# medical-genomics-group/rs-bann

Hardware: AMD Instinct MI355X
Metric: HMC leapfrog steps/sec (whole node), 50k indiv × 500k SNP × 1k branches (higher is better)
Workload: dtype 2-bit genotype codes x f32 params (i8 MFMA digits, exact int32 accumulate, f32 head); 1 GPU; c3: 1000 branches x 500 SNPs, n=50000, D=1 W=4 S=4, RidgeARD, tanh, Izmailov step sizes; n=50000, snps=500000, branches=1000, branches_per_gpu=1000, parallelism=branch-shard x1

## Files before the change

include/bann.h:

```cpp
#ifndef BANN_H
#define BANN_H

#include <stdint.h>

#ifdef __cplusplus
extern "C" {
#endif

typedef struct bann_ctx bann_ctx;

typedef enum {
  BANN_OK = 0,
  BANN_E_HIP = -1,
  BANN_E_SHAPE = -2,
  BANN_E_OOM = -3,
  BANN_E_STATE = -4,
  BANN_E_ARG = -5
} bann_status;

typedef enum { BANN_TANH = 0, BANN_RELU = 1, BANN_LEAKY_RELU = 2, BANN_SILU = 3, BANN_IDENTITY = 4 } bann_activation;

typedef enum {
  BANN_RIDGE_ARD = 0,
  BANN_RIDGE_BASE = 1,
// ... 136 lines not shown
int bann_residual_to_target(bann_ctx* ctx, int32_t b);
int bann_residual_from_target(bann_ctx* ctx, int32_t b, double* sum, double* sumsq);
int bann_rebuild_targets(bann_ctx* ctx, const int32_t* branches, int32_t nb, const float* residual_device);


int bann_gibbs_posterior(bann_ctx* ctx, const int32_t* branches, int32_t nb, const float* hyper, double* shape_out,
                         double* scale_out, double* out_stat_out);
int bann_gibbs_sample_precisions(bann_ctx* ctx, const int32_t* branches, int32_t nb, const float* hyper,
                                 float output_precision, float error_precision, uint64_t seed);
int bann_get_params_all(bann_ctx* ctx, float* out);


int bann_arch_layer_widths(int32_t m, int32_t depth, int32_t hidden_rule, int32_t hidden_fixed, float hidden_fraction,
                           int32_t summary_rule, int32_t summary_fixed, float summary_fraction,
                           int32_t* layer_widths_out);

typedef struct {
  int32_t mode;
  float variance, gamma_shape, gamma_scale;
  int32_t num_effective;
  float proportion_effective;
  int32_t has_fixed_precision;  float fixed_precision;
} bann_init_cfg;
int bann_init_branches(bann_ctx* ctx, const int32_t* branches, int32_t nb, const bann_init_cfg* cfg, uint64_t seed);


typedef int (*bann_allreduce_fn)(void* user, void* host_buf, int64_t count, int32_t dtype);

int bann_shard_branches(const int32_t* marker_counts, int32_t nbranches, int32_t world, int32_t* starts_out);
int bann_comm_unique_id(uint8_t* id_out);
int bann_ctx_comm_init(bann_ctx* ctx, const uint8_t* id, int32_t nranks, int32_t rank);
int bann_ctx_comm_callback(bann_ctx* ctx, bann_allreduce_fn fn, void* user, int32_t nranks, int32_t rank);
int bann_comm_info(const bann_ctx* ctx, int32_t* kind, int32_t* nranks, int32_t* rank, int32_t* backend_ranks);
int bann_residual_update_host(bann_allreduce_fn fn, void* user, float* local_delta, float* residual, int64_t n);
int bann_exchange_residual(bann_ctx* ctx, float* residual_host);
int bann_exchange_residual_device(bann_ctx* ctx);
int bann_network_hmc_step(bann_ctx* ctx, const float* y, float bias, float lambda_e, int32_t L,
                          float max_hamiltonian_error, int32_t step_mode, float step_factor, const float* eps,
                          const float* momentum, uint64_t seed, const float* u, int32_t* status_out,
                          double* h_trace_out, double* rss_out);
int bann_set_network_step_rule(bann_ctx* ctx, int32_t common_mode, float tau);
int bann_set_network_adapt_trajectories(bann_ctx* ctx, int32_t k);
int bann_network_step_rule_state(const bann_ctx* ctx, int32_t* mode, int32_t* adapted, int32_t* frozen);
int bann_network_info(const bann_ctx* ctx, int32_t* group_rows);
int bann_network_step_rule_info(const bann_ctx* ctx, double* out4);

int bann_branch_kernel_path(const bann_ctx* ctx, int32_t b);
const char* bann_fused_kernel_name(void);
int bann_set_hidden_gemm_bf16(bann_ctx* ctx, int32_t enabled);
int bann_set_graph_replay(bann_ctx* ctx, int32_t enabled);
int bann_get_graph_replay(const bann_ctx* ctx);
int bann_set_fused_enabled(bann_ctx* ctx, int32_t enabled);
int64_t bann_packed_genotype_bytes(const bann_ctx* ctx);

#ifdef __cplusplus
}
#endif
#endif
```

rs-bann_amd/bann/_lib.py:

```python
from __future__ import annotations

import ctypes as C
import os

HERE = os.path.dirname(os.path.abspath(__file__))
PKG_ROOT = os.path.dirname(HERE)
REPO_ROOT = os.path.dirname(PKG_ROOT)
LIB_PATH = os.environ.get("BANN_LIB") or os.path.join(PKG_ROOT, "librsbann_amd.so")
HEADER_PATH = os.path.join(REPO_ROOT, "include", "bann.h")
HEADER_PATHS = [HEADER_PATH, os.path.join(REPO_ROOT, "include", "bann_net.h")]

BANN_OK = 0
STATUS = {0: "BANN_OK", -1: "BANN_E_HIP", -2: "BANN_E_SHAPE", -3: "BANN_E_OOM", -4: "BANN_E_STATE",
          -5: "BANN_E_ARG"}
ACTIVATIONS = {"tanh": 0, "relu": 1, "leaky_relu": 2, "silu": 3, "identity": 4}
PRIORS = {"ridge_ard": 0, "ridge_base": 1, "lasso_ard": 2, "lasso_base": 3, "std_normal": 4}
STEP_MODES = {"uniform": 0, "random": 1, "std_scaled": 2, "izmailov": 3, "injected": 100}
HMC_STATUS = {0: "accepted", 1: "rejected", 2: "rejected_early"}


class BannLibraryError(RuntimeError):
    pass


# ... 115 lines not shown
    "bann_exchange_residual_device": (C.c_int, [_P]),
    "bann_set_network_step_rule": (C.c_int, [_P, _i32, _f32]),
    "bann_network_step_rule_info": (C.c_int, [_P, _pf64]),
    "bann_set_network_adapt_trajectories": (C.c_int, [_P, _i32]),
    "bann_network_info": (C.c_int, [_P, C.POINTER(C.c_int32)]),
    "bann_network_step_rule_state": (C.c_int, [_P, C.POINTER(C.c_int32), C.POINTER(C.c_int32), C.POINTER(C.c_int32)]),
    "bann_residual_set": (C.c_int, [_P, _pf32]),
    "bann_residual_get": (C.c_int, [_P, _pf32]),
    "bann_residual_device": (C.c_int, [_P, C.POINTER(_pf32)]),
    "bann_residual_init": (C.c_int, [_P, _pf32, _f32, _pf64, _pf64]),
    "bann_residual_stats": (C.c_int, [_P, _pf64, _pf64]),
    "bann_residual_shift": (C.c_int, [_P, _f32, _pf64, _pf64]),
    "bann_residual_to_target": (C.c_int, [_P, _i32]),
    "bann_residual_from_target": (C.c_int, [_P, _i32, _pf64, _pf64]),
    "bann_rebuild_targets": (C.c_int, [_P, _pi32, _i32, _P]),
    "bann_set_launch_timing": (C.c_int, [_P, _i32]),
    "bann_launch_timing": (C.c_int, [_P, _pf32, _pf32, _pi32, _i32]),
    "bann_network_timing": (C.c_int, [_P, _pf32, _pf32, _pi32, _i32]),
    "bann_ctx_num_individuals": (_i64, [_P]),
    "bann_leapfrog_begin": (C.c_int, [_P, _pi32, _i32, _i32, _f32, _i32, _f32, _u64]),
    "bann_leapfrog_steps": (C.c_int, [_P, _i32]),
    "bann_leapfrog_end": (C.c_int, [_P, _pi32, _pi32]),
    "bann_leapfrog_predictions_device": (C.c_int, [_P, C.POINTER(_pf32)]),
    "bann_leapfrog_residual_delta_device": (C.c_int, [_P, _P]),
    "bann_leapfrog_residual_delta": (C.c_int, [_P, _P]),
    "bann_fused_kernel_name": (C.c_char_p, []),
    "bann_branch_get_step_sizes": (C.c_int, [_P, C.c_int32, _P]),
    "bann_predict_many": (C.c_int, [_P, _P, C.c_int32, _P]),
    "bann_synchronize": (C.c_int, [_P]),
    "bann_gibbs_posterior": (C.c_int, [_P, _pi32, _i32, _pf32, _pf64, _pf64, _pf64]),
    "bann_gibbs_sample_precisions": (C.c_int, [_P, _pi32, _i32, _pf32, _f32, _f32, _u64]),
    "bann_get_params_all": (C.c_int, [_P, _pf32]),
    "bann_arch_layer_widths": (C.c_int, [_i32, _i32, _i32, _i32, _f32, _i32, _i32, _f32, _pi32]),
    "bann_init_branches": (C.c_int, [_P, _pi32, _i32, C.POINTER(InitCfg), _u64]),
    "bann_phen_stats_write": (C.c_int, [C.c_char_p, _f32, _f32, _f32]),
    "bann_net_init": (C.c_int, [_P, C.POINTER(InitCfg), _u64]),
    "bann_net_simulate_y": (C.c_int, [_P, _P, _f32, _u64, _pf32, _pf32]),
    "bann_net_write_params": (C.c_int, [_P, C.c_char_p]),
    "bann_models_reserve": (C.c_int, [_P, _i32]),
    "bann_models_capacity": (C.c_int, [_P]),
    "bann_models_pass_width": (C.c_int, []),
    "bann_models_set_params": (C.c_int, [_P, _i32, _i32, _pf32]),
    "bann_models_set_bias": (C.c_int, [_P, _i32, _f32]),
    "bann_models_predict": (C.c_int, [_P, _i32, _i32, _pf32, _pf32, _pf32]),
    "bann_models_branch_predictions": (C.c_int, [_P, _i32, _pi32, _i32, _pf32]),
    "bann_models_stats_pass_width": (C.c_int, []),
    "bann_models_branch_stats": (C.c_int, [_P, _i32, _i32, _pi32, _i32, _pf32, _pf64, _pf32, _pf32, _pf32]),
    "bann_models_branch_stats_timed": (C.c_int, [_P, _i32, _i32, _pi32, _i32, _pf32, _pf64, _pf32, _pf32]),
    "bann_profile_session": (C.c_int, [_P, _i32, _pf32, _pf32]),
    "bann_branch_kernel_path": (C.c_int, [_P, _i32]),
    "bann_set_fused_enabled": (C.c_int, [_P, _i32]),
    "bann_set_hidden_gemm_bf16": (C.c_int, [_P, _i32]),
    "bann_packed_genotype_bytes": (_i64, [_P]),
    "bann_net_create": (C.c_int, [_P, C.POINTER(PrecisionHyperparams), _u64, C.POINTER(_P)]),
    "bann_net_destroy": (C.c_int, [_P]),
    "bann_net_set_rng_hooks": (C.c_int, [_P, C.POINTER(RngHooks)]),
    "bann_net_set_global": (C.c_int, [_P, _f32, _f32, _f32, _f32]),
    "bann_net_train": (C.c_int, [_P, _pf32, _i64, C.POINTER(McmcCfg), C.c_char_p]),
    "bann_net_train_single_branch": (C.c_int, [_P, _pf32, _i64, C.POINTER(McmcCfg), C.c_char_p]),
    "bann_net_train_network": (C.c_int, [_P, _pf32, _i64, C.POINTER(McmcCfg), _i32, C.c_char_p]),
    "bann_net_network_timing": (C.c_int, [_P, _pf64]),
    "bann_net_perturb": (C.c_int, [_P, _i32, _f32, _i32, _f32]),
    "bann_net_predict": (C.c_int, [_P, _P, _pf32]),
    "bann_net_predict_models": (C.c_int, [_P, _P, C.POINTER(C.c_char_p), _i32, _pf32, _pf32, _pf32]),
    "bann_net_rss": (C.c_int, [_P, _P, _pf32, _i64, _pf64]),
    "bann_net_gradient": (C.c_int, [_P, _P, _pf32, _i64, _pf32]),
    "bann_net_branch_r2s": (C.c_int, [_P, _P, _pf32, _i64, _pf32]),
    "bann_net_activations": (C.c_int, [_P, _P, _i32, _pf32]),
    "bann_net_population_effect_sizes": (C.c_int, [_P, _P, _pf32]),
    "bann_net_branch_r2s_models": (C.c_int, [_P, _P, C.POINTER(C.c_char_p), _i32, _pf32, _i64, _pf32]),
    "bann_net_population_effect_sizes_models": (C.c_int, [_P, _P, C.POINTER(C.c_char_p), _i32, _pf32, _pf32, _pf32]),
    "bann_net_summary": (C.c_int, [_P, C.POINTER(TrainSummary)]),
    "bann_net_records": (C.c_int, [_P, _pf32, _pf32, _i32]),
    "bann_net_residual": (C.c_int, [_P, _pf32]),
    "bann_net_set_test_data": (C.c_int, [_P, _P, _pf32, _i64]),
    "bann_net_records_test": (C.c_int, [_P, _pf32, _i32]),
    "bann_set_trajectory_recording": (C.c_int, [_P, _i32]),
    "bann_branch_get_trajectory": (C.c_int, [_P, _i32, _i32, _pi32, _pf32, _pf32, _pf64]),
    "bann_branch_get_trajectory_joint": (C.c_int, [_P, _i32, _i32, _pi32, _pf32, _pf32, _pf32, _pf64]),
    "bann_set_graph_replay": (C.c_int, [_P, _i32]),
    "bann_get_graph_replay": (C.c_int, [_P]),
    "bann_net_save": (C.c_int, [_P, C.c_char_p]),
    "bann_net_load": (C.c_int, [_P, C.c_char_p]),
    "bann_net_last_error": (C.c_char_p, [_P]),
}

_lib = None


def load_library(path: str = LIB_PATH):
    global _lib
    if _lib is not None:
        return _lib
    if not os.path.exists(path):
        raise BannLibraryError(
            f"{path} not found: build the HIP library first (python -c 'import __graft_entry__ as g; g.build()' "
            "or make -C rs-bann_amd/csrc).  There is no CPU fallback.")
    lib = C.CDLL(path)
    for name, (res, args) in SIGNATURES.items():
        fn = getattr(lib, name)
        fn.restype = res
        fn.argtypes = args
    _lib = lib
    return lib
```

rs-bann_amd/csrc/kernel_util.h:

```cpp
#pragma once
#include <hip/hip_runtime.h>
#include <stdint.h>

#include "bann_internal.h"

typedef int v4i __attribute__((ext_vector_type(4)));
typedef float v4f __attribute__((ext_vector_type(4)));

struct HeadLds {
  float W[BANN_MAXL][4][4];
  float bias[BANN_MAXL][4];
};

__device__ __forceinline__ float wave_sum(float v) {
#pragma unroll
  for (int o = 32; o > 0; o >>= 1) v += __shfl_xor(v, o);
  return v;
}
__device__ __forceinline__ double wave_sum_d(double v) {
#pragma unroll
  for (int o = 32; o > 0; o >>= 1) v += __shfl_xor(v, o);
  return v;
}

#define LDS_BARRIER()                                      \
  do {                                                     \
    asm volatile("s_waitcnt lgkmcnt(0)" ::: "memory");     \
    __builtin_amdgcn_s_barrier();                          \
    asm volatile("" ::: "memory");                         \
  } while (0)

typedef __attribute__((address_space(3))) void* lds_ptr_t;

__device__ __forceinline__ uint32_t lds_off(const void* p) { return (uint32_t)(uintptr_t)p; }
__device__ __forceinline__ void glds16(const void* gsrc, const void* lds_dst) {
  const uint32_t m0 = __builtin_amdgcn_readfirstlane(lds_off(lds_dst));
#ifndef BANN_GLDS_NT
#define BANN_GLDS_NT 1
#endif
#if BANN_GLDS_NT
  asm volatile("s_mov_b32 m0, %0\n\ts_nop 0\n\tglobal_load_lds_dwordx4 %1, off nt" ::"s"(m0), "v"(gsrc) : "memory", "m0");
#else
  asm volatile("s_mov_b32 m0, %0\n\ts_nop 0\n\tglobal_load_lds_dwordx4 %1, off" ::"s"(m0), "v"(gsrc) : "memory", "m0");
#endif
}
__device__ __forceinline__ void glds16_s(const void* sbase, uint32_t voff, const void* lds_dst) {
  const uint32_t m0 = __builtin_amdgcn_readfirstlane(lds_off(lds_dst));
#if BANN_GLDS_NT
  asm volatile("s_mov_b32 m0, %0\n\ts_nop 0\n\tglobal_load_lds_dwordx4 %1, %2 nt" ::"s"(m0), "v"(voff), "s"(sbase)
               : "memory", "m0");
#else
  asm volatile("s_mov_b32 m0, %0\n\ts_nop 0\n\tglobal_load_lds_dwordx4 %1, %2" ::"s"(m0), "v"(voff), "s"(sbase)
               : "memory", "m0");
#endif
}
__device__ __forceinline__ void glds4(const void* gsrc, const void* lds_dst) {
  const uint32_t m0 = __builtin_amdgcn_readfirstlane(lds_off(lds_dst));
  asm volatile("s_mov_b32 m0, %0\n\ts_nop 0\n\tglobal_load_lds_dword %1, off" ::"s"(m0), "v"(gsrc) : "memory", "m0");
}
__device__ __forceinline__ void lds_st_f32(float* p, float v) {
  asm volatile("ds_write_b32 %0, %1" ::"v"(lds_off(p)), "v"(v) : "memory");
}
__device__ __forceinline__ void lds_st_v4f(v4f* p, v4f v) {
  asm volatile("ds_write_b128 %0, %1" ::"v"(lds_off(p)), "v"(v) : "memory");
}

__device__ __forceinline__ uint32_t fbits(float x) { return __builtin_bit_cast(uint32_t, x); }
__device__ __forceinline__ float fpow2(uint32_t biased_exp) { return __builtin_bit_cast(float, biased_exp << 23); }

typedef unsigned short v2u16 __attribute__((ext_vector_type(2)));
__device__ __forceinline__ uint32_t max_u16x2(uint32_t a, uint32_t b) {
  return __builtin_bit_cast(uint32_t, __builtin_elementwise_max(__builtin_bit_cast(v2u16, a), __builtin_bit_cast(v2u16, b)));
}
__device__ __forceinline__ uint32_t wave_max_u16x2(uint32_t v) {
  v = max_u16x2(v, (uint32_t)__builtin_amdgcn_update_dpp((int)v, (int)v, 0xB1, 0xF, 0xF, false));
  v = max_u16x2(v, (uint32_t)__builtin_amdgcn_update_dpp((int)v, (int)v, 0x4E, 0xF, 0xF, false));
  v = max_u16x2(v, (uint32_t)__builtin_amdgcn_update_dpp((int)v, (int)v, 0x141, 0xF, 0xF, false));
  v = max_u16x2(v, (uint32_t)__builtin_amdgcn_update_dpp((int)v, (int)v, 0x140, 0xF, 0xF, false));
  v = max_u16x2(v, (uint32_t)__builtin_amdgcn_update_dpp((int)v, (int)v, 0x142, 0xA, 0xF, false));
  v = max_u16x2(v, (uint32_t)__builtin_amdgcn_update_dpp((int)v, (int)v, 0x143, 0xC, 0xF, false));
  return (uint32_t)__builtin_amdgcn_readlane((int)v, 63);
}

typedef int v2i __attribute__((ext_vector_type(2)));
typedef __attribute__((address_space(3))) v2i lds_v2i;
__device__ __forceinline__ v4i lds_tr8_pair(const char* p0, const char* p1) {
  const v2i a = __builtin_amdgcn_ds_read_tr8_b64_v2i32((lds_v2i*)(p0));
  const v2i b = __builtin_amdgcn_ds_read_tr8_b64_v2i32((lds_v2i*)(p1));
  return v4i{a.x, a.y, b.x, b.y};
}

__device__ __forceinline__ uint32_t digits4(float v) {
  uint32_t w = 0;
#pragma unroll
  for (int d = 0; d < 4; ++d) {
    const float r = __builtin_rintf(v);
    w |= ((uint32_t)(int)r & 0xFFu) << (8 * d);
    v = (v - r) * 128.f;
  }
  return w;
}
```

rs-bann_amd/csrc/kernels_fx.hip:

```cpp
#include <stdlib.h>
#include <type_traits>

#include "activations.h"
#include "bann_internal.h"
#include "fx_shapes.h"
#include "kernel_util.h"
#include "update_core.h"

#define FX_WAVES 4
#define FX_SLOT 8192

#ifndef FX_STAMPS
#define FX_STAMPS 0
#endif
#ifndef FXT_PD
#define FXT_PD 12
#endif
#ifndef FX_ABL
#define FX_ABL 0
#endif
#if FX_STAMPS
#define FX_STAMP(i)                                            \
  do {                                                         \
    const unsigned long long t_ = __builtin_amdgcn_s_memtime(); \
    ph[i] += t_ - t_last;                                      \
    t_last = t_;                                               \
  } while (0)
#else
#define FX_STAMP(i) \
  do {              \
  } while (0)
#endif
#if FX_ABL & 8
#define FX_MFMA(a, b, c) ((c) + ((a) ^ (b)))
#else
#define FX_MFMA(a, b, c) __builtin_amdgcn_mfma_i32_16x16x64_i8((a), (b), (c), 0, 0, 0)
#endif

typedef unsigned int v4u __attribute__((ext_vector_type(4)));

#define FX_ONES3 (v4i{0, 0, 0, 0x40404040})

__device__ __forceinline__ void fx_fwd_chunk(v4i A, v4u X, v4i (&facc)[4]) {
  facc[0] = __builtin_amdgcn_mfma_i32_16x16x64_i8(A, (v4i)(X & 0x03030303u), facc[0], 0, 0, 0);
  facc[1] = __builtin_amdgcn_mfma_i32_16x16x64_i8(A, (v4i)(X & 0x0F0F0F0Fu), facc[1], 0, 0, 0);
  facc[2] = __builtin_amdgcn_mfma_i32_16x16x64_i8(A, (v4i)(X & 0x3F3F3F3Fu), facc[2], 0, 0, 0);
  facc[3] = __builtin_amdgcn_mfma_i32_16x16x64_i8(A, (v4i)X, facc[3], 0, 0, 0);
}
__device__ __forceinline__ void fx_fwd_fields(v4i (&facc)[4]) {
  facc[3] -= facc[2];
  facc[2] -= facc[1];
  facc[1] -= facc[0];
}
__device__ __forceinline__ v4i fx_rowsum64_acc(v4i A, v4i acc) {
  return __builtin_amdgcn_mfma_i32_16x16x64_i8(A, v4i{0x40404040, 0x40404040, 0x40404040, 0x40404040}, acc, 0, 0, 0);
}
__device__ __forceinline__ v4i fx_bwd_unpack(uint32_t wv) {
  return v4i{(int)(wv & 0x03030303u), (int)(wv & 0x0C0C0C0Cu), (int)(wv & 0x30303030u), (int)(wv & 0xC0C0C0C0u)};
}

__device__ __forceinline__ float ufl(float v) {
  return __builtin_bit_cast(float, __builtin_amdgcn_readfirstlane(__builtin_bit_cast(int, v)));
}

__device__ __forceinline__ void vm_wait(int k) {
  switch (k) {
    case 2: asm volatile("s_waitcnt vmcnt(2)" ::: "memory"); break;
    case 3: asm volatile("s_waitcnt vmcnt(3)" ::: "memory"); break;
    case 4: asm volatile("s_waitcnt vmcnt(4)" ::: "memory"); break;
    case 5: asm volatile("s_waitcnt vmcnt(5)" ::: "memory"); break;
    case 6: asm volatile("s_waitcnt vmcnt(6)" ::: "memory"); break;
    case 7: asm volatile("s_waitcnt vmcnt(7)" ::: "memory"); break;
// ... 52 lines not shown
                    int32_t* __restrict__ upd_cnt, const FoldJob* __restrict__ folds) {
  constexpr int NH = NL - 1;
  constexpr int NW = FX_WAVES;
  constexpr int NS = 8 + (NH - 1) * 20;
  __shared__ __attribute__((aligned(16))) char s_x[NW][2][FX_SLOT];
  __shared__ __attribute__((aligned(16))) char s_dig[NW][4 * FX_DROW];
  __shared__ __attribute__((aligned(16))) float s_y[NW][2][64];
  __shared__ __attribute__((aligned(16))) char s_w0[8 * 1024];
  __shared__ __attribute__((aligned(16))) float s_hw[NL][20];
  __shared__ float s_hs[NW][NS];
  __shared__ double s_rss[NW];

  const GradItem it = items[blockIdx.x];
  const int b = it.branch;
  const BranchDev& bd = st.br[b];
  const int wave = __builtin_amdgcn_readfirstlane(threadIdx.x >> 6);
  const int lane = threadIdx.x & 63;
  const int nch = NCH ? NCH : bd.nchunks;
  const int64_t n = st.n;
  const int tb = it.frag_begin >> 2, te = (it.frag_end + 3) >> 2;

  const int g = lane >> 4, i16 = lane & 15, tq = i16 >> 1, tp = lane & 1;
  const int gsw = g & 1;
  const uint32_t fo0 = (uint32_t)((16 * g + tq + 8 * gsw) * 16 + 8 * (tp ^ gsw));
  const uint32_t fo1 = (uint32_t)((16 * g + tq + 8 * (1 ^ gsw)) * 16 + 8 * (tp ^ 1 ^ gsw));
  const int pe = i16, po = (i16 + 8) & 15;
  const uint32_t boe = (uint32_t)(pe * 16 + 4 * (2 * ((g >> 1) ^ (pe >> 3)) + (g & 1)));
  const uint32_t boo = (uint32_t)(po * 16 + 4 * (2 * ((g >> 1) ^ (po >> 3)) + (g & 1)));
  const int iota = 4 * i16 + g;
  char* const sd = &s_dig[wave][0];
  char* const sd_w = sd + (i16 >> 2) * FX_DROW + (4 * g + (i16 & 3)) * 16;
  const char* const sd_r = sd + g * FX_DROW + tq * 16 + 8 * tp;
  const bool net_err = st.nete != nullptr;
  const float* ybr = net_err ? st.nete : st.y + bd.y_off;
  float* predb = st.pred + bd.y_off;
  const int64_t tile_bytes = (int64_t)nch * 1024;
  const uint64_t xb = (uint64_t)(uintptr_t)(reinterpret_cast<const char*>(st.xu2) + bd.x_off);
  const char* xbase_s = reinterpret_cast<const char*>(
      ((uint64_t)(uint32_t)__builtin_amdgcn_readfirstlane((int)(uint32_t)(xb >> 32)) << 32) |
      (uint32_t)__builtin_amdgcn_readfirstlane((int)(uint32_t)xb));

  const bool pad_row = 64 * (nch - 1) + 16 * (lane >> 4) + (((lane & 15) - 8 * ((lane >> 4) & 1)) & 15) >= bd.m;
  auto issue_chunk = [&](int tt, int sl, int c) {
    if (FX_ABL & 16) return;
    if (c == nch - 1 && pad_row) return;
    glds16_s(xbase_s + (uint64_t)tt * (uint64_t)tile_bytes + (uint64_t)(c * 1024), (uint32_t)lane * 16u,
             &s_x[wave][sl][c * 1024]);
  };
  auto issue_y = [&](int tt, int sl) {
    if (FX_ABL & 16) return;
    const int64_t row = 64 * (int64_t)tt + iota;
    glds4(ybr + (row < n ? row : n - 1), &s_y[wave][sl][0]);
  };
  int tt = tb + wave, sl = 0;
  if (tt < te) {
    for (int c = 0; c < nch; ++c) issue_chunk(tt, 0, c);
    issue_y(tt, 0);
    if (tt + NW < te) {
      for (int c = 0; c < nch; ++c) issue_chunk(tt + NW, 1, c);
      issue_y(tt + NW, 1);
    }
  }
  const float* th = st.theta + bd.p_off;
  for (int t = threadIdx.x; t < NL * 20; t += 64 * NW) {
    const int l = t / 20, r = t - l * 20;
    float v = 0.f;
    if (r < 16) {
      const int j = r >> 2, k = r & 3;
      if (l >= 1 && j < bd.win[l] && k < bd.widths[l]) v = th[bd.woff[l] + k * bd.win[l] + j];
    } else {
      const int k = r - 16;
      if (l == 0 && k < bd.widths[0]) v = st.fc[b].c0[k];
      if (l >= 1 && l < NH && k < bd.widths[l]) v = th[bd.boff[l] + k];
    }
    s_hw[l][r] = v;
  }
  float zscale = st.fc[b].scale[g];
  for (int c = wave; c < nch; c += NW)
    *reinterpret_cast<v4i*>(&s_w0[c * 1024 + lane * 16]) =
        *reinterpret_cast<const v4i*>(st.dig + bd.dig_off + ((int64_t)c * 64 + lane) * 16);
  asm volatile("s_waitcnt vmcnt(0)" ::: "memory");
  asm volatile("" : "+v"(zscale));
  __syncthreads();
  v4i rowsum64 = v4i{0, 0, 0, 0};
  for (int c = 0; c < nch; ++c) rowsum64 = fx_rowsum64_acc(*reinterpret_cast<const v4i*>(&s_w0[c * 1024 + lane * 16]), rowsum64);
  float uW[NL][4][4], uB[NH][4];
#pragma unroll
  for (int l = 0; l < NL; ++l) {
#pragma unroll
    for (int j = 0; j < 4; ++j)
#pragma unroll
      for (int k = 0; k < 4; ++k)
        uW[l][j][k] = (l >= 1 && (l < NL - 1 || k == 0)) ? sgpr_f(s_hw[l][4 * j + k]) : 0.f;
    if (l < NH)
#pragma unroll
      for (int k = 0; k < 4; ++k) uB[l][k] = sgpr_f(s_hw[l][16 + k]);
  }


  v4i acc[32];
#pragma unroll
  for (int u = 0; u < 32; ++u) acc[u] = v4i{0, 0, 0, 0};
  v4i acc3 = v4i{0, 0, 0, 0};
  int R[4] = {0, 0, 0, 0};
  double rss = 0.0;
  float db[NH][4], dWo[4];
  float dW[NL > 2 ? NL - 2 : 1][4][4];
#pragma unroll
  for (int k = 0; k < 4; ++k) {
    dWo[k] = 0.f;
#pragma unroll
    for (int l = 0; l < NH; ++l) db[l][k] = 0.f;
#pragma unroll
    for (int l = 0; l < (NL > 2 ? NL - 2 : 1); ++l)
#pragma unroll
      for (int j = 0; j < 4; ++j) dW[l][j][k] = 0.f;
  }

#if FX_STAMPS
  unsigned long long ph[8] = {0, 0, 0, 0, 0, 0, 0, 0}, ntl = 0;
  const unsigned long long rt0 = __builtin_amdgcn_s_memrealtime(), mt0 = __builtin_amdgcn_s_memtime();
  unsigned long long t_last = mt0;
#endif
  for (; tt < te; tt += NW, sl ^= 1) {
    const bool more = tt + NW < te;
    const bool more2 = tt + 2 * NW < te;
    FX_STAMP(5);
    vm_wait(more ? nch + 1 : 0);
    FX_STAMP(0);
    const char* xs = &s_x[wave][sl][0];

    v4i facc[4] = {v4i{0, 0, 0, 0}, v4i{0, 0, 0, 0}, v4i{0, 0, 0, 0}, rowsum64};
    __builtin_amdgcn_s_setprio(1);
    {
      constexpr int FD = 2;
      v4u Xq[FD];
      v4i Aq[FD];
#pragma unroll
      for (int c = 0; c < FD; ++c) {
        Xq[c] = v4u{0u, 0u, 0u, 0u};
        Aq[c] = v4i{0, 0, 0, 0};
        if (NCH != 0 || c < nch) {
          Xq[c] = (v4u)lds_tr8_pair(xs + c * 1024 + fo0, xs + c * 1024 + fo1);
          Aq[c] = *reinterpret_cast<const v4i*>(&s_w0[c * 1024 + lane * 16]);
        }
      }
#pragma unroll
      for (int c = 0; c < 8; ++c) {
        if (NCH == 0 && c >= nch) continue;
        const v4u Xc = Xq[c % FD];
        const v4i Ac = Aq[c % FD];
        if (c + FD < 8 && (NCH != 0 || c + FD < nch)) {
          Xq[c % FD] = (v4u)lds_tr8_pair(xs + (c + FD) * 1024 + fo0, xs + (c + FD) * 1024 + fo1);
          Aq[c % FD] = *reinterpret_cast<const v4i*>(&s_w0[(c + FD) * 1024 + lane * 16]);
        }
#if FX_ABL & 1
        const v4i B0 = (v4i)Xc, B1 = (v4i)Xc, B2 = (v4i)Xc, B3 = (v4i)Xc;
#else
        const v4i B0 = (v4i)(Xc & 0x03030303u);
        const v4i B1 = (v4i)(Xc & 0x0F0F0F0Fu);
        const v4i B2 = (v4i)(Xc & 0x3F3F3F3Fu);
        const v4i B3 = (v4i)Xc;
#endif
        facc[0] = FX_MFMA(Ac, B0, facc[0]);
        facc[1] = FX_MFMA(Ac, B1, facc[1]);
        facc[2] = FX_MFMA(Ac, B2, facc[2]);
        facc[3] = FX_MFMA(Ac, B3, facc[3]);
        __builtin_amdgcn_sched_barrier(0);
      }
    }
    __builtin_amdgcn_sched_barrier(0);
    FX_STAMP(1);
    __builtin_amdgcn_s_setprio(1);
    fx_fwd_fields(facc);
    float z0 = zscale * comb4(facc[0]), z1 = (0.25f * zscale) * comb4(facc[1]);
    float z2 = (0.0625f * zscale) * comb4(facc[2]), z3 = (0.015625f * zscale) * comb4(facc[3]);
    swap32(z0, z2);
    swap32(z1, z3);
    swap16(z0, z1);
    swap16(z2, z3);

    const int64_t row = 64 * (int64_t)tt + iota;
    const bool valid = row < n;
    const float yv = s_y[wave][sl][lane];
    float d[4];
#if FX_ABL & 4
    d[0] = z0 + yv, d[1] = z1, d[2] = z2, d[3] = z3;
    if (write_pred && valid) predb[row] = z0;
    rss += (double)z1;
#else
    {
      const auto& Wh = uW;
      const auto& Bh = uB;
      float z[NH][4], a[NH][4];
      z[0][0] = z0 + Bh[0][0];
      z[0][1] = z1 + Bh[0][1];
      z[0][2] = z2 + Bh[0][2];
      z[0][3] = z3 + Bh[0][3];
#pragma unroll
      for (int k = 0; k < 4; ++k) a[0][k] = act_h_t<ACT>(z[0][k]);
#pragma unroll
      for (int l = 1; l < NH; ++l) {
#pragma unroll
        for (int k = 0; k < 4; ++k) {
          float s = Bh[l][k];
#pragma unroll
          for (int j = 0; j < 4; ++j) s = fmaf(a[l - 1][j], Wh[l][j][k], s);
          z[l][k] = s;
          a[l][k] = act_h_t<ACT>(s);
        }
      }
      float out = 0.f;
#pragma unroll
      for (int j = 0; j < 4; ++j) out = fmaf(a[NH - 1][j], Wh[NL - 1][j][0], out);
      const float e = valid ? (net_err ? yv : out - yv) : 0.f;
      if (write_pred && valid) predb[row] = out;
      rss += (double)e * (double)e;
      float err[4];
#pragma unroll
      for (int j = 0; j < 4; ++j) {
        dWo[j] = fmaf(a[NH - 1][j], e, dWo[j]);
        err[j] = e * Wh[NL - 1][j][0];
      }
#pragma unroll
      for (int l = NH - 1; l >= 0; --l) {
        float dl[4];
#pragma unroll
        for (int k = 0; k < 4; ++k) {
          dl[k] = act_dh_t<ACT>(z[l][k], a[l][k]) * err[k];
          db[l][k] += dl[k];
        }
        if (l >= 1) {
#pragma unroll
          for (int j = 0; j < 4; ++j) {
            float sj = 0.f;
#pragma unroll
            for (int k = 0; k < 4; ++k) {
              dW[l - 1][j][k] = fmaf(a[l - 1][j], dl[k], dW[l - 1][j][k]);
              sj = fmaf(dl[k], Wh[l][j][k], sj);
            }
            err[j] = sj;
          }
        } else {
#pragma unroll
          for (int k = 0; k < 4; ++k) d[k] = dl[k];
        }
      }
    }
#endif

    if (more2) {
      asm volatile("" ::"v"(yv));
      issue_y(tt + 2 * NW, sl);
    }
    __builtin_amdgcn_sched_barrier(0);
    FX_STAMP(2);
    constexpr int PD = FXT_PD;
    uint32_t wq[PD];
#pragma unroll
    for (int u = 0; u < PD; ++u)
      wq[u] = (NCH != 0 || u < 4 * nch) ? *reinterpret_cast<const uint32_t*>(xs + 256 * u + ((u & 1) ? boo : boe)) : 0u;
    int dl[4] = {0, 0, 0, 0};
    bool grow = false;
    {
      bool lane_need = false;
#pragma unroll
      for (int k = 0; k < 4; ++k) {
        const int ek = (int)((fbits(d[k]) >> 23) & 0xFFu);
        lane_need |= ek > (R[k] ? R[k] : 5);
      }
      if (__builtin_amdgcn_ballot_w64(lane_need) != 0) {
        const uint32_t e01 = wave_max_u16x2(((fbits(d[0]) >> 23) & 0xFFu) | (((fbits(d[1]) >> 23) & 0xFFu) << 16));
        const uint32_t e23 = wave_max_u16x2(((fbits(d[2]) >> 23) & 0xFFu) | (((fbits(d[3]) >> 23) & 0xFFu) << 16));
        const int E[4] = {(int)(e01 & 0xFFFFu), (int)(e01 >> 16), (int)(e23 & 0xFFFFu), (int)(e23 >> 16)};
#pragma unroll
        for (int k = 0; k < 4; ++k) {
          if (E[k] >= 6 && (R[k] == 0 || E[k] > R[k])) {
            if (R[k] != 0) {
              dl[k] = E[k] + 2 - R[k];
              grow = true;
            }
            R[k] = E[k] + 2;
          }
        }
      }
    }
    if (grow) {
      const int sh = g == 0 ? dl[0] : g == 1 ? dl[1] : g == 2 ? dl[2] : dl[3];
#pragma unroll
      for (int u = 0; u < 32; ++u)
        if (NCH != 0 || u < 4 * nch) acc[u] = shr_digits(acc[u], sh);
      acc3 = shr_digits(acc3, sh);
    }
    v4u w;
    const int kslot_sh = 2 * g;
#pragma unroll
    for (int k = 0; k < 4; ++k) w[k] = digits4_fx(d[k], 153 - kslot_sh - (R[k] ? R[k] : 255));
    *reinterpret_cast<v4u*>(sd_w) = w;

    __builtin_amdgcn_sched_barrier(0);
    FX_STAMP(3);
    __builtin_amdgcn_s_setprio(0);
    const v4i A = lds_tr8_pair(sd_r, sd_r + 8 * 16);
    acc3 = FX_MFMA(A, FX_ONES3, acc3);
    {
      auto unpack = [](uint32_t wv) -> v4i {
#if FX_ABL & 2
        return v4i{(int)wv, (int)wv, (int)wv, (int)wv};
#else
        return fx_bwd_unpack(wv);
#endif
      };
      v4i Bn = unpack(wq[0]), Bn2 = unpack(wq[1]);
#pragma unroll
      for (int u = 0; u < 32; ++u) {
        if (NCH == 0 && u >= 4 * nch) continue;
        const v4i Bv = Bn;
        Bn = Bn2;
        if (u + 2 < 32 && (NCH != 0 || u + 2 < 4 * nch)) Bn2 = unpack(wq[(u + 2) % PD]);
        if (more2 && (u & 3) == 1) {
          asm volatile("" ::"v"(Bn2[0]), "v"(Bn2[1]), "v"(Bn2[2]), "v"(Bn2[3]));
          issue_chunk(tt + 2 * NW, sl, u >> 2);
        }
        if (u + PD < 32 && (NCH != 0 || u + PD < 4 * nch))
          wq[u % PD] = *reinterpret_cast<const uint32_t*>(xs + 256 * (u + PD) + (((u + PD) & 1) ? boo : boe));
        acc[u] = FX_MFMA(A, Bv, acc[u]);
      }
    }
    FX_STAMP(4);
#if FX_STAMPS
    ++ntl;
#endif
  }
  asm volatile("s_waitcnt vmcnt(0)" ::: "memory");
#if FX_STAMPS
  ph[6] = __builtin_amdgcn_s_memrealtime() - rt0;
  ph[7] = __builtin_amdgcn_s_memtime() - mt0;
  if (lane == 0 && st.dbg) {
    for (int i = 0; i < 8; ++i) atomicAdd(&st.dbg[i], ph[i]);
    atomicAdd(&st.dbg[15], ntl);
  }
#endif

  {
    const double rs = wave_sum_d(rss);
    float hs[NS];
#pragma unroll
    for (int k = 0; k < 4; ++k) {
      hs[k] = wave_sum(db[0][k]);
      hs[4 + k] = wave_sum(dWo[k]);
    }
#pragma unroll
    for (int l = 1; l < NH; ++l)
#pragma unroll
      for (int k = 0; k < 4; ++k) {
        hs[8 + (l - 1) * 20 + k] = wave_sum(db[l][k]);
#pragma unroll
        for (int j = 0; j < 4; ++j) hs[8 + (l - 1) * 20 + 4 + 4 * j + k] = wave_sum(dW[l - 1][j][k]);
      }
    if (lane == 0) {
      s_rss[wave] = rs;
#pragma unroll
      for (int q = 0; q < NS; ++q) s_hs[wave][q] = hs[q];
    }
  }
  __syncthreads();
  {
    const int Rl = g == 0 ? R[0] : g == 1 ? R[1] : g == 2 ? R[2] : R[3];
    float* red = reinterpret_cast<float*>(&s_x[wave][0][0]);
#pragma unroll
    for (int u = 0; u < 32; ++u)
      if (u < 4 * nch) red[u * 64 + lane] = Rl ? __builtin_amdgcn_ldexpf(comb4_exact2(acc[u], acc3), Rl - 153) : 0.f;
  }
  __syncthreads();
  float* part = st.part + it.part_at;
  const bool pub = UPD && upd_cnt != nullptr && (folds != nullptr || bd.nsplits > 1);
  auto pst = [&](float* a, float v) {
    if (pub)
      __hip_atomic_store(a, v, __ATOMIC_RELAXED, __HIP_MEMORY_SCOPE_AGENT);
    else
      *a = v;
  };
  float db0[4];
#pragma unroll
  for (int k = 0; k < 4; ++k) db0[k] = (s_hs[0][k] + s_hs[1][k]) + (s_hs[2][k] + s_hs[3][k]);
  const int m = bd.m;
// ... 54 lines not shown
        if (threadIdx.x == 0) {
          __builtin_amdgcn_fence(__ATOMIC_ACQUIRE, "agent");
          asm volatile("s_waitcnt vmcnt(0)" ::: "memory");
          upd_cnt[b] = 0;
        }
        __syncthreads();
      }
      if (folds) {
        fold_solo_all<64 * FX_WAVES>(st, folds[it.fold_ix], bd);
        __syncthreads();
      }
      float* s_th = reinterpret_cast<float*>(&s_x[0][0][0]);
      update_small<64 * FX_WAVES, 1, 2>(st, b, bd, upd_mode, false, upd_step, s_redd, s_th);
    }
  }
}

template <int NL, int NCH, int UPD>
static void launch_fx_nlu(const DevState& st, const GradItem* items, int32_t nitems, int act, int wp, int um, int us,
                          int32_t* cnt, const FoldJob* fo, hipStream_t s) {
  const dim3 grid((unsigned)nitems), block(64 * FX_WAVES);
  switch (act) {
    case 0: hipLaunchKernelGGL((k_fused_grad_fx<NL, 0, NCH, UPD>), grid, block, 0, s, st, items, wp, um, us, cnt, fo); break;
    case 1: hipLaunchKernelGGL((k_fused_grad_fx<NL, 1, NCH, UPD>), grid, block, 0, s, st, items, wp, um, us, cnt, fo); break;
    case 2: hipLaunchKernelGGL((k_fused_grad_fx<NL, 2, NCH, UPD>), grid, block, 0, s, st, items, wp, um, us, cnt, fo); break;
    case 3: hipLaunchKernelGGL((k_fused_grad_fx<NL, 3, NCH, UPD>), grid, block, 0, s, st, items, wp, um, us, cnt, fo); break;
    default: hipLaunchKernelGGL((k_fused_grad_fx<NL, 4, NCH, UPD>), grid, block, 0, s, st, items, wp, um, us, cnt, fo); break;
  }
}
template <int NL, int NCH>
static void launch_fx_nl(const DevState& st, const GradItem* items, int32_t nitems, int act, int wp, int um, int us,
                         int32_t* cnt, const FoldJob* fo, hipStream_t s) {
  if (cnt)
    launch_fx_nlu<NL, NCH, 1>(st, items, nitems, act, wp, um, us, cnt, fo, s);
  else
    launch_fx_nlu<NL, NCH, 0>(st, items, nitems, act, wp, um, us, nullptr, nullptr, s);
}

void launch_fused_grad_fx(const DevState& st, const GradItem* items, int32_t nitems, int32_t L, int32_t act,
                          int full8, int write_pred, int upd_mode, int upd_step, int32_t* upd_cnt,
                          const FoldJob* folds, hipStream_t s) {
  if (nitems <= 0) return;
  const int wp = write_pred, um = upd_mode, us = upd_step;
  const FoldJob* fo = upd_cnt ? folds : nullptr;
  switch (L * 2 + (full8 ? 1 : 0)) {
    case 4: launch_fx_nl<2, 0>(st, items, nitems, act, wp, um, us, upd_cnt, fo, s); break;
    case 5: launch_fx_nl<2, 8>(st, items, nitems, act, wp, um, us, upd_cnt, fo, s); break;
    case 6: launch_fx_nl<3, 0>(st, items, nitems, act, wp, um, us, upd_cnt, fo, s); break;
    case 7: launch_fx_nl<3, 8>(st, items, nitems, act, wp, um, us, upd_cnt, fo, s); break;
    case 8: launch_fx_nl<4, 0>(st, items, nitems, act, wp, um, us, upd_cnt, fo, s); break;
    case 9: launch_fx_nl<4, 8>(st, items, nitems, act, wp, um, us, upd_cnt, fo, s); break;
    default: break;
  }
}

constexpr int FWD_NU = 3;
__device__ __forceinline__ void vm_wait_n(int k) {
#define VMW(i) \
  case i: asm volatile("s_waitcnt vmcnt(" #i ")" ::: "memory"); break;
  switch (k) {
    VMW(1) VMW(2) VMW(3) VMW(4) VMW(5) VMW(6) VMW(7) VMW(8) VMW(9) VMW(10) VMW(11) VMW(12) VMW(13) VMW(14)
    VMW(15) VMW(16) VMW(17) VMW(18) VMW(19) VMW(20) VMW(21) VMW(22) VMW(23) VMW(24) VMW(25) VMW(26) VMW(27)
    VMW(28) VMW(29) VMW(30) VMW(31)
    default: asm volatile("s_waitcnt vmcnt(0)" ::: "memory"); break;
  }
#undef VMW
}

template <int NL, int ACT, int NCH, int NU>
__global__ void __launch_bounds__(64 * FX_WAVES, 2)
    k_forward_fx(DevState st, const GradItem* __restrict__ items) {
  constexpr int NH = NL - 1;
  constexpr int NW = FX_WAVES;
  constexpr int NS = 2;
  static_assert(NU == 0 || NCH == 8, "the half-tile ring needs 8-chunk tiles");
  __shared__ __attribute__((aligned(16))) char s_x[NW][NU > 0 ? 1 : NS][NU > 0 ? NU * 4096 : FX_SLOT];
  __shared__ __attribute__((aligned(16))) char s_w0[NU > 0 ? 16 : 8 * 1024];
  __shared__ __attribute__((aligned(16))) float s_hw[NL][20];

  const GradItem it = items[blockIdx.x];
  const int b = it.branch;
  const BranchDev& bd = st.br[b];
  const int wave = __builtin_amdgcn_readfirstlane(threadIdx.x >> 6);
  const int lane = threadIdx.x & 63;
  const int nch = NCH ? NCH : bd.nchunks;
  const int64_t n = st.n;
  const int tb = it.frag_begin >> 2, te = (it.frag_end + 3) >> 2;

  const float* th = st.theta + bd.p_off;
  for (int t = threadIdx.x; t < NL * 20; t += 64 * NW) {
    const int l = t / 20, r = t - l * 20;
    float v = 0.f;
    if (r < 16) {
      const int j = r >> 2, k = r & 3;
      if (l >= 1 && j < bd.win[l] && k < bd.widths[l]) v = th[bd.woff[l] + k * bd.win[l] + j];
    } else {
      const int k = r - 16;
      if (l == 0 && k < bd.widths[0]) v = st.fc[b].c0[k];
      if (l >= 1 && l < NH && k < bd.widths[l]) v = th[bd.boff[l] + k];
    }
    s_hw[l][r] = v;
  }
  const int g = lane >> 4, i16 = lane & 15, tq = i16 >> 1, tp = lane & 1;
  float zscale = st.fc[b].scale[g];
  v4i Areg[NU > 0 ? 8 : 1];
  if constexpr (NU > 0) {
// ... 1284 lines not shown
```

Baseline: 822.7 leapfrog steps/s.

## Split fused grad loop into steady-state and edge tiles with immediate-offset DMA

Splits the per-wave tile loop of the fused fixed-point gradient kernel into a steady-state path, where all rows are valid and prefetch is guaranteed, and an edge path for the tail. The steady path drops bounds checks, prediction writes and row clamping, and issues the next tile's global-to-LDS loads with a scalar base plus compile-time immediate offsets instead of per-chunk address computation. Per-group exponent ranges are tracked in registers to simplify the rescale check. A probe kernel and API are added to verify that the immediate offset also advances the LDS destination on this hardware. The cost is more code and register pressure, plus a dependence on that hardware behaviour being correct.

```diff
diff --git a/include/bann.h b/include/bann.h
--- a/include/bann.h
+++ b/include/bann.h
@@ -212,6 +212,7 @@
 int bann_get_graph_replay(const bann_ctx* ctx);
 int bann_set_fused_enabled(bann_ctx* ctx, int32_t enabled);
 int64_t bann_packed_genotype_bytes(const bann_ctx* ctx);
+int bann_fx_dma_offset_probe(int32_t* lds_follows, int32_t* built_mode);
 
 #ifdef __cplusplus
 }
diff --git a/rs-bann_amd/bann/_lib.py b/rs-bann_amd/bann/_lib.py
--- a/rs-bann_amd/bann/_lib.py
+++ b/rs-bann_amd/bann/_lib.py
@@ -191,6 +191,7 @@
     "bann_set_fused_enabled": (C.c_int, [_P, _i32]),
     "bann_set_hidden_gemm_bf16": (C.c_int, [_P, _i32]),
     "bann_packed_genotype_bytes": (_i64, [_P]),
+    "bann_fx_dma_offset_probe": (C.c_int, [_pi32, _pi32]),
     "bann_net_create": (C.c_int, [_P, C.POINTER(PrecisionHyperparams), _u64, C.POINTER(_P)]),
     "bann_net_destroy": (C.c_int, [_P]),
     "bann_net_set_rng_hooks": (C.c_int, [_P, C.POINTER(RngHooks)]),
diff --git a/rs-bann_amd/csrc/kernel_util.h b/rs-bann_amd/csrc/kernel_util.h
--- a/rs-bann_amd/csrc/kernel_util.h
+++ b/rs-bann_amd/csrc/kernel_util.h
@@ -54,6 +54,33 @@
                : "memory", "m0");
 #endif
 }
+template <int OFF>
+__device__ __forceinline__ void glds16_so(const void* sbase, uint32_t voff, uint32_t m0v) {
+  static_assert(OFF >= 0 && OFF < 4096, "13-bit signed immediate, used non-negative");
+#if BANN_GLDS_NT
+  asm volatile("s_nop 0\n\tglobal_load_lds_dwordx4 %0, %1 offset:%c2 nt" ::"v"(voff), "s"(sbase), "n"(OFF), "{m0}"(m0v)
+               : "memory");
+#else
+  asm volatile("s_nop 0\n\tglobal_load_lds_dwordx4 %0, %1 offset:%c2" ::"v"(voff), "s"(sbase), "n"(OFF), "{m0}"(m0v)
+               : "memory");
+#endif
+}
+template <int OFF>
+__device__ __forceinline__ void glds16_so_masked(const void* sbase, uint32_t voff, uint32_t m0v, uint64_t mask) {
+  static_assert(OFF >= 0 && OFF < 4096, "13-bit signed immediate, used non-negative");
+  uint64_t keep;
+#if BANN_GLDS_NT
+  asm volatile("s_mov_b64 %0, exec\n\ts_mov_b64 exec, %5\n\tglobal_load_lds_dwordx4 %1, %2 offset:%c3 nt\n\ts_mov_b64 exec, %0"
+               : "=&s"(keep)
+               : "v"(voff), "s"(sbase), "n"(OFF), "{m0}"(m0v), "s"(mask)
+               : "memory");
+#else
+  asm volatile("s_mov_b64 %0, exec\n\ts_mov_b64 exec, %5\n\tglobal_load_lds_dwordx4 %1, %2 offset:%c3\n\ts_mov_b64 exec, %0"
+               : "=&s"(keep)
+               : "v"(voff), "s"(sbase), "n"(OFF), "{m0}"(m0v), "s"(mask)
+               : "memory");
+#endif
+}
 __device__ __forceinline__ void glds4(const void* gsrc, const void* lds_dst) {
   const uint32_t m0 = __builtin_amdgcn_readfirstlane(lds_off(lds_dst));
   asm volatile("s_mov_b32 m0, %0\n\ts_nop 0\n\tglobal_load_lds_dword %1, off" ::"s"(m0), "v"(gsrc) : "memory", "m0");
diff --git a/rs-bann_amd/csrc/kernels_fx.hip b/rs-bann_amd/csrc/kernels_fx.hip
--- a/rs-bann_amd/csrc/kernels_fx.hip
+++ b/rs-bann_amd/csrc/kernels_fx.hip
@@ -1,6 +1,7 @@
 #include <stdlib.h>
 #include <type_traits>
 
+#include "../../include/bann.h"
 #include "activations.h"
 #include "bann_internal.h"
 #include "fx_shapes.h"
@@ -18,6 +19,21 @@
 #endif
 #ifndef FX_ABL
 #define FX_ABL 0
+#endif
+#ifndef FX_STEADY
+#define FX_STEADY 1
+#endif
+#ifndef FX_DMA_IMM
+#define FX_DMA_IMM (FX_STEADY ? 2 : 0)
+#endif
+#if FX_DMA_IMM != 0 && FX_DMA_IMM != 2
+#error "FX_DMA_IMM: 0 or 2"
+#endif
+#ifndef FX_RFB
+#define FX_RFB FX_STEADY
+#endif
+#ifndef FXT_PD_EDGE
+#define FXT_PD_EDGE 4
 #endif
 #if FX_STAMPS
 #define FX_STAMP(i)                                            \
@@ -176,6 +192,37 @@
     const int64_t row = 64 * (int64_t)tt + iota;
     glds4(ybr + (row < n ? row : n - 1), &s_y[wave][sl][0]);
   };
+#if FX_STEADY
+  auto issue_y_full = [&](int tt, int sl) {
+    if (FX_ABL & 16) return;
+    glds4(ybr + (64 * (int64_t)tt + iota), &s_y[wave][sl][0]);
+  };
+#if FX_DMA_IMM
+  const uint64_t live_rows = __builtin_amdgcn_ballot_w64(!pad_row);
+  auto issue_piece = [&](const char* nb, uint32_t lb, int c) __attribute__((always_inline)) {
+    if (FX_ABL & 16) return;
+    const char* gb = nb + 4096 * (c >> 2);
+    const uint32_t voff = (uint32_t)lane * 16u;
+    const uint32_t m0v = lb + 4096u * (uint32_t)(c >> 2);
+    if (NCH != 0 && c != NCH - 1) {
+      switch (c & 3) {
+        case 0: glds16_so<0>(gb, voff, m0v); break;
+        case 1: glds16_so<1024>(gb, voff, m0v); break;
+        case 2: glds16_so<2048>(gb, voff, m0v); break;
+        default: glds16_so<3072>(gb, voff, m0v); break;
+      }
+    } else {
+      const uint64_t mk = (NCH != 0 || c == nch - 1) ? live_rows : ~0ull;
+      switch (c & 3) {
+        case 0: glds16_so_masked<0>(gb, voff, m0v, mk); break;
+        case 1: glds16_so_masked<1024>(gb, voff, m0v, mk); break;
+        case 2: glds16_so_masked<2048>(gb, voff, m0v, mk); break;
+        default: glds16_so_masked<3072>(gb, voff, m0v, mk); break;
+      }
+    }
+  };
+#endif
+#endif
   int tt = tb + wave, sl = 0;
   if (tt < te) {
     for (int c = 0; c < nch; ++c) issue_chunk(tt, 0, c);
@@ -246,9 +293,20 @@
   const unsigned long long rt0 = __builtin_amdgcn_s_memrealtime(), mt0 = __builtin_amdgcn_s_memtime();
   unsigned long long t_last = mt0;
 #endif
+#if FX_RFB
+  int Rg[4] = {5, 5, 5, 5};
+  int Rd[4] = {255, 255, 255, 255};
+#endif
+#if FX_STEADY
+  auto tile = [&](auto steady_c) __attribute__((always_inline)) {
+    constexpr bool ST = decltype(steady_c)::value;
+#else
   for (; tt < te; tt += NW, sl ^= 1) {
-    const bool more = tt + NW < te;
-    const bool more2 = tt + 2 * NW < te;
+    constexpr bool ST = false;
+#endif
+    const bool more = ST || tt + NW < te;
+    const bool more2 = ST || tt + 2 * NW < te;
+    const bool wpred = !ST && write_pred;
     FX_STAMP(5);
     vm_wait(more ? nch + 1 : 0);
     FX_STAMP(0);
@@ -305,12 +363,12 @@
     swap16(z2, z3);
 
     const int64_t row = 64 * (int64_t)tt + iota;
-    const bool valid = row < n;
+    const bool valid = ST || row < n;
     const float yv = s_y[wave][sl][lane];
     float d[4];
 #if FX_ABL & 4
     d[0] = z0 + yv, d[1] = z1, d[2] = z2, d[3] = z3;
-    if (write_pred && valid) predb[row] = z0;
+    if (wpred && valid) predb[row] = z0;
     rss += (double)z1;
 #else
     {
@@ -338,7 +396,7 @@
 #pragma unroll
       for (int j = 0; j < 4; ++j) out = fmaf(a[NH - 1][j], Wh[NL - 1][j][0], out);
       const float e = valid ? (net_err ? yv : out - yv) : 0.f;
-      if (write_pred && valid) predb[row] = out;
+      if (wpred && valid) predb[row] = out;
       rss += (double)e * (double)e;
       float err[4];
 #pragma unroll
@@ -375,11 +433,20 @@
 
     if (more2) {
       asm volatile("" ::"v"(yv));
-      issue_y(tt + 2 * NW, sl);
-    }
+#if FX_STEADY
+      if (ST)
+        issue_y_full(tt + 2 * NW, sl);
+      else
+#endif
+        issue_y(tt + 2 * NW, sl);
+    }
+#if FX_STEADY && FX_DMA_IMM
+    const char* const nb = xbase_s + (uint64_t)(tt + 2 * NW) * (uint64_t)tile_bytes;
+    const uint32_t lb = __builtin_amdgcn_readfirstlane(lds_off(&s_x[wave][sl][0]));
+#endif
     __builtin_amdgcn_sched_barrier(0);
     FX_STAMP(2);
-    constexpr int PD = FXT_PD;
+    constexpr int PD = ST || !FX_STEADY ? FXT_PD : FXT_PD_EDGE;
     uint32_t wq[PD];
 #pragma unroll
     for (int u = 0; u < PD; ++u)
@@ -391,7 +458,11 @@
 #pragma unroll
       for (int k = 0; k < 4; ++k) {
         const int ek = (int)((fbits(d[k]) >> 23) & 0xFFu);
+#if FX_RFB
+        lane_need |= ek > Rg[k];
+#else
         lane_need |= ek > (R[k] ? R[k] : 5);
+#endif
       }
       if (__builtin_amdgcn_ballot_w64(lane_need) != 0) {
         const uint32_t e01 = wave_max_u16x2(((fbits(d[0]) >> 23) & 0xFFu) | (((fbits(d[1]) >> 23) & 0xFFu) << 16));
@@ -399,6 +470,15 @@
         const int E[4] = {(int)(e01 & 0xFFFFu), (int)(e01 >> 16), (int)(e23 & 0xFFFFu), (int)(e23 >> 16)};
 #pragma unroll
         for (int k = 0; k < 4; ++k) {
+#if FX_RFB
+          if (E[k] > Rg[k]) {
+            if (Rg[k] != 5) {
+              dl[k] = E[k] + 2 - Rg[k];
+              grow = true;
+            }
+            Rg[k] = Rd[k] = E[k] + 2;
+          }
+#else
           if (E[k] >= 6 && (R[k] == 0 || E[k] > R[k])) {
             if (R[k] != 0) {
               dl[k] = E[k] + 2 - R[k];
@@ -406,6 +486,7 @@
             }
             R[k] = E[k] + 2;
           }
+#endif
         }
       }
     }
@@ -418,8 +499,13 @@
     }
     v4u w;
     const int kslot_sh = 2 * g;
+#if FX_RFB
+#pragma unroll
+    for (int k = 0; k < 4; ++k) w[k] = digits4_fx(d[k], 153 - kslot_sh - Rd[k]);
+#else
 #pragma unroll
     for (int k = 0; k < 4; ++k) w[k] = digits4_fx(d[k], 153 - kslot_sh - (R[k] ? R[k] : 255));
+#endif
     *reinterpret_cast<v4u*>(sd_w) = w;
 
     __builtin_amdgcn_sched_barrier(0);
@@ -444,7 +530,12 @@
         if (u + 2 < 32 && (NCH != 0 || u + 2 < 4 * nch)) Bn2 = unpack(wq[(u + 2) % PD]);
         if (more2 && (u & 3) == 1) {
           asm volatile("" ::"v"(Bn2[0]), "v"(Bn2[1]), "v"(Bn2[2]), "v"(Bn2[3]));
-          issue_chunk(tt + 2 * NW, sl, u >> 2);
+#if FX_STEADY && FX_DMA_IMM
+          if (ST)
+            issue_piece(nb, lb, u >> 2);
+          else
+#endif
+            issue_chunk(tt + 2 * NW, sl, u >> 2);
         }
         if (u + PD < 32 && (NCH != 0 || u + PD < 4 * nch))
           wq[u % PD] = *reinterpret_cast<const uint32_t*>(xs + 256 * (u + PD) + (((u + PD) & 1) ? boo : boe));
@@ -455,7 +546,21 @@
 #if FX_STAMPS
     ++ntl;
 #endif
-  }
+#if FX_STEADY
+  };
+  {
+    const int64_t t_full = (n >> 6) - 2 * NW, t_more = (int64_t)te - 2 * NW;
+    const int t_st = write_pred ? tt : (int)(t_full < t_more ? t_full : t_more);
+    for (; tt < t_st; tt += NW, sl ^= 1) tile(std::true_type{});
+  }
+  for (; tt < te; tt += NW, sl ^= 1) tile(std::false_type{});
+#else
+  }
+#endif
+#if FX_RFB
+#pragma unroll
+  for (int k = 0; k < 4; ++k) R[k] = Rg[k] != 5 ? Rg[k] : 0;
+#endif
   asm volatile("s_waitcnt vmcnt(0)" ::: "memory");
 #if FX_STAMPS
   ph[6] = __builtin_amdgcn_s_memrealtime() - rt0;
@@ -616,6 +721,46 @@
     case 9: launch_fx_nl<4, 8>(st, items, nitems, act, wp, um, us, upd_cnt, fo, s); break;
     default: break;
   }
+}
+
+__global__ void __launch_bounds__(64) k_glds_offset_probe(const char* __restrict__ src, uint32_t* __restrict__ dst) {
+  __shared__ __attribute__((aligned(16))) uint32_t s_p[1024];
+  for (int i = threadIdx.x; i < 1024; i += 64) s_p[i] = 0xFFFFFFFFu;
+  __syncthreads();
+  const uint32_t m0v = __builtin_amdgcn_readfirstlane(lds_off(&s_p[0]));
+  const uint32_t voff = threadIdx.x * 16u;
+  glds16_so<0>(src, voff, m0v);
+  glds16_so<1024>(src, voff, m0v);
+  glds16_so<2048>(src, voff, m0v);
+  glds16_so<3072>(src, voff, m0v);
+  asm volatile("s_waitcnt vmcnt(0)" ::: "memory");
+  __syncthreads();
+  for (int i = threadIdx.x; i < 1024; i += 64) dst[i] = s_p[i];
+}
+
+extern "C" int bann_fx_dma_offset_probe(int32_t* lds_follows, int32_t* built_mode) {
+  if (!lds_follows || !built_mode) return BANN_E_ARG;
+  *built_mode = FX_STEADY ? FX_DMA_IMM : 0;
+  *lds_follows = -1;
+  uint32_t h_src[1024], h_dst[1024];
+  for (int i = 0; i < 1024; ++i) h_src[i] = 0x9E3779B1u * (uint32_t)(i + 1) & 0x7FFFFFFFu;
+  void *d_src = nullptr, *d_dst = nullptr;
+  bool ok = hipMalloc(&d_src, 4096) == hipSuccess && hipMalloc(&d_dst, 4096) == hipSuccess &&
+            hipMemcpy(d_src, h_src, 4096, hipMemcpyHostToDevice) == hipSuccess;
+  if (ok) {
+    hipLaunchKernelGGL(k_glds_offset_probe, dim3(1), dim3(64), 0, nullptr, (const char*)d_src, (uint32_t*)d_dst);
+    ok = hipGetLastError() == hipSuccess && hipMemcpy(h_dst, d_dst, 4096, hipMemcpyDeviceToHost) == hipSuccess;
+  }
+  if (d_src) (void)hipFree(d_src);
+  if (d_dst) (void)hipFree(d_dst);
+  if (!ok) return BANN_E_HIP;
+  bool both = true, global_only = true;
+  for (int i = 0; i < 1024; ++i) {
+    both = both && h_dst[i] == h_src[i];
+    global_only = global_only && h_dst[i] == (i < 256 ? h_src[768 + i] : 0xFFFFFFFFu);
+  }
+  *lds_follows = both ? 1 : global_only ? 0 : -1;
+  return BANN_OK;
 }
 
 constexpr int FWD_NU = 3;
```

After: 831.7 leapfrog steps/s (median of 6 runs). 1.01x the previous value.
